# esa-prl/planning-motion_planning

Measured on AMD Instinct MI355X. Metric: Eikonal Gcells/s + ms-to-path, 4k² & 16k² costmap at 1/2/4/8 GPU, higher is better.
Workload: dtype f64; 1 GPU; C2: 4096x4096 DEM-derived cost raster, single goal, FIM on 1 MI355X; H=4096, W=4096, split=1x1, tile=64, parallelism=single-gpu

## Files before the change

planning-motion_planning_amd/csrc/eik_common.hpp:

```cpp
#pragma once
#include <hip/hip_runtime.h>
#include <stdint.h>

namespace eik {

constexpr int kTile = 64;
constexpr int kThreads = 256;
constexpr int kLds = kTile + 2;

template <typename R> struct Real;
template <> struct Real<float> {
    using U = unsigned int;
    static __host__ __device__ constexpr float inf() { return __builtin_inff(); }
};
template <> struct Real<double> {
    using U = unsigned long long;
    static __host__ __device__ constexpr double inf() { return __builtin_inf(); }
};

__device__ __forceinline__ double eik_ref(double thor, double tver, double c) {
#pragma clang fp contract(off)
    const double inf = Real<double>::inf();
    if (thor == inf) return tver == inf ? inf : tver + c;
    if (tver == inf) return thor + c;
    const double d = thor - tver;
    if (c < __builtin_fabs(d)) return __builtin_fmin(thor, tver) + c;
    return 0.5 * (thor + tver + __builtin_sqrt(2.0 * (c * c) - d * d));
}

__device__ __forceinline__ double solve3_ref(double v0, double v1, double v2, double C) {
#pragma clang fp contract(off)
    const double C2 = C * C;
    const bool m1 = v1 > v0;
    const double t01 = m1 ? v1 : v0;
    const bool m2 = v2 > t01;
    const double tmax = m2 ? v2 : t01;
    const int im = m2 ? 2 : (m1 ? 1 : 0);
    const double d0 = tmax - v0, d1 = tmax - v1, d2 = tmax - v2;
    const bool ok3 = C2 > (d0 * d0 + d1 * d1) + d2 * d2;
    const double u0 = im == 0 ? v1 : v0, u1 = im == 2 ? v1 : v2;
    const bool n1 = u1 > u0;
    const double t2 = n1 ? u1 : u0;
    const double e0 = t2 - u0, e1 = t2 - u1;
    const bool ok2 = C2 > e0 * e0 + e1 * e1;
    const double w = n1 ? u0 : u1;
    const double dw = w - w;
    const bool ok1 = C2 > dw * dw;
    double S, Q, nn;
    if (ok3) {
        S = v0 + (v1 + v2);
        Q = v0 * v0 + (v1 * v1 + v2 * v2);
        nn = 3.0;
    } else if (ok2) {
        S = u0 + u1;
        Q = u0 * u0 + u1 * u1;
        nn = 2.0;
    } else {
        S = w;
        Q = w * w;
        nn = 1.0;
    }
    const double tr = (S + __builtin_sqrt((nn * C2 + S * S) - nn * Q)) / nn;
    return (ok3 || ok2 || ok1) ? tr : Real<double>::inf();
}

template <typename R>
__device__ __forceinline__ R godunov2(R a, R b, R c) {
    const R lo = a < b ? a : b;
    const R hi = a < b ? b : a;
    const R d = hi - lo;
    const R t1 = lo + c;
    const R t2 = R(0.5) * (lo + hi + __builtin_sqrt(R(2) * (c * c) - d * d));
    return (hi == Real<R>::inf() || c < d) ? t1 : t2;
}
template <>
__device__ __forceinline__ float godunov2<float>(float a, float b, float c) {
    const float lo = fminf(a, b), hi = fmaxf(a, b);
    const float d = hi - lo;
    const float t1 = lo + c;
    const float t2 = 0.5f * (lo + hi + __builtin_amdgcn_sqrtf(2.f * (c * c) - d * d));
    return (hi == Real<float>::inf() || c < d) ? t1 : t2;
}

__device__ __forceinline__ float umin(float a, float b) {
    return __uint_as_float(min(__float_as_uint(a), __float_as_uint(b)));
}
__device__ __forceinline__ float umax(float a, float b) {
    return __uint_as_float(max(__float_as_uint(a), __float_as_uint(b)));
}
__device__ __forceinline__ double umin(double a, double b) {
    const unsigned long long x = __double_as_longlong(a), y = __double_as_longlong(b);
    return __longlong_as_double(x < y ? x : y);
}
__device__ __forceinline__ double umax(double a, double b) {
    const unsigned long long x = __double_as_longlong(a), y = __double_as_longlong(b);
    return __longlong_as_double(x < y ? y : x);
}

__device__ __forceinline__ float godunov2_step(float a, float b, float c) {
    const float lo = umin(a, b), hi = umax(a, b);
    const float d = hi - lo;
    const float t2 = lo + 0.5f * (d + __builtin_amdgcn_sqrtf(2.f * (c * c) - d * d));
    return c < d ? lo + c : t2;
}
__device__ __forceinline__ double godunov2_step(double a, double b, double c) {
    const double lo = umin(a, b), hi = umax(a, b);
    const double d = hi - lo;
    const double t2 = lo + 0.5 * (d + __builtin_sqrt(2.0 * (c * c) - d * d));
    return c < d ? lo + c : t2;
}

__device__ __forceinline__ float godunov2_fast(float a, float b, float c) {
    const float lo = umin(a, b), hi = umax(a, b);
    const float d = umin(hi - lo, c);
    const float c2 = c * c;
    const float q = __builtin_fmaf(-d, d, c2) + c2;
    return __builtin_fmaf(0.5f, d + __builtin_amdgcn_sqrtf(q), lo);
}
__device__ __forceinline__ double godunov2_fast(double a, double b, double c) {
    const double lo = umin(a, b), hi = umax(a, b);
    const double d = umin(hi - lo, c);
    const double c2 = c * c;
    const double q = __builtin_fma(-d, d, c2) + c2;
    return __builtin_fma(0.5, d + __builtin_sqrt(q), lo);
}

#ifndef EIK_CHAIN
#define EIK_CHAIN 3
#endif
__device__ __forceinline__ float godunov2_chain(float a, float b, float c, float c2x2) {
    const float lo = umin(a, b);
    const float diff = a - b;
    float d;
    asm("v_min_f32 %0, |%1|, %2" : "=v"(d) : "v"(diff), "v"(c));
    const float q = __builtin_fmaf(-d, d, c2x2);
    return __builtin_fmaf(0.5f, d + __builtin_amdgcn_sqrtf(q), lo);
}
__device__ __forceinline__ double fmin_nn(double a, double b) {
    double r;
    asm("v_min_f64 %0, %1, %2" : "=v"(r) : "v"(a), "v"(b));
    return r;
}
__device__ __forceinline__ double sqrt_sweep(double q) {
#if EIK_CHAIN
    const double qc = q;
#else
    double qc;
    asm("v_max_f64 %0, %1, %2" : "=v"(qc) : "v"(q), "v"(0x1p-1000));
#endif
    const double y = __builtin_amdgcn_rsq(qc);
    double g = qc * y, h = 0.5 * y;
    const double r = __builtin_fma(-h, g, 0.5);
    g = __builtin_fma(g, r, g);
    h = __builtin_fma(h, r, h);
    const double e = __builtin_fma(-g, g, qc);
    return __builtin_fma(e, h, g);
}
__device__ __forceinline__ double godunov2_chain(double a, double b, double c, double c2x2) {
    const double lo = fmin_nn(a, b);
    const double diff = a - b;
    double d;
    asm("v_min_f64 %0, |%1|, %2" : "=v"(d) : "v"(diff), "v"(c));
    const double q = __builtin_fma(-d, d, c2x2);
#if EIK_CHAIN >= 3
    const double base = __builtin_fma(0.5, d, lo);
    const double y = __builtin_amdgcn_rsq(q);
    const double g = q * y, h = 0.5 * y;
    const double s1 = __builtin_fma(__builtin_fma(-g, g, q), h, g);
    const double e2 = __builtin_fma(-s1, s1, q);
    return __builtin_fma(0.5, __builtin_fma(e2, h, s1), base);
#elif EIK_CHAIN >= 2
    const double base = __builtin_fma(0.5, d, lo);
    const double y = __builtin_amdgcn_rsq(q);
    const double g = q * y, h = 0.5 * y, hq = 0.25 * y;
    const double r = __builtin_fma(-h, g, 0.5);
    const double g1 = __builtin_fma(g, r, g);
    const double e = __builtin_fma(-g1, g1, q);
    return __builtin_fma(e, hq, __builtin_fma(0.5, g1, base));
#elif EIK_CHAIN
    return __builtin_fma(0.5, sqrt_sweep(q), __builtin_fma(0.5, d, lo));
#else
    return __builtin_fma(0.5, d + sqrt_sweep(q), lo);
#endif
}

__device__ __forceinline__ float wave_shr1(float v) {
    return __int_as_float(__builtin_amdgcn_update_dpp(0, __float_as_int(v), 0x138, 0xF, 0xF, false));
}
__device__ __forceinline__ float wave_shr1(float v, float lane0) {
    return __int_as_float(__builtin_amdgcn_update_dpp(__float_as_int(lane0), __float_as_int(v), 0x138, 0xF, 0xF, false));
}
__device__ __forceinline__ double wave_shr1(double v, double lane0) {
    const unsigned long long u = __double_as_longlong(v), o = __double_as_longlong(lane0);
    const int lo = __builtin_amdgcn_update_dpp((int)(o & 0xffffffffu), (int)(u & 0xffffffffu), 0x138, 0xF, 0xF, false);
    const int hi = __builtin_amdgcn_update_dpp((int)(o >> 32), (int)(u >> 32), 0x138, 0xF, 0xF, false);
    return __longlong_as_double(((unsigned long long)(unsigned)hi << 32) | (unsigned)lo);
}
__device__ __forceinline__ double wave_shr1(double v) {
    const unsigned long long u = __double_as_longlong(v);
    const int lo = __builtin_amdgcn_update_dpp(0, (int)(u & 0xffffffffu), 0x138, 0xF, 0xF, false);
    const int hi = __builtin_amdgcn_update_dpp(0, (int)(u >> 32), 0x138, 0xF, 0xF, false);
    return __longlong_as_double(((unsigned long long)(unsigned)hi << 32) | (unsigned)lo);
}

__device__ __forceinline__ float wave_shr1_umin_id(float v) {
    return __int_as_float(__builtin_amdgcn_update_dpp(-1, __float_as_int(v), 0x138, 0xF, 0xF, false));
}
__device__ __forceinline__ double wave_shr1_umin_id(double v) {
    const unsigned long long u = __double_as_longlong(v);
    const int lo = __builtin_amdgcn_update_dpp(-1, (int)(u & 0xffffffffu), 0x138, 0xF, 0xF, false);
    const int hi = __builtin_amdgcn_update_dpp(-1, (int)(u >> 32), 0x138, 0xF, 0xF, false);
    return __longlong_as_double(((unsigned long long)(unsigned)hi << 32) | (unsigned)lo);
}

__device__ __forceinline__ void lds_min(float* p, float v) {
    atomicMin(reinterpret_cast<unsigned int*>(p), __float_as_uint(v));
}
__device__ __forceinline__ void lds_min(double* p, double v) {
    atomicMin(reinterpret_cast<unsigned long long*>(p), (unsigned long long)__double_as_longlong(v));
}

}
```

planning-motion_planning_amd/csrc/fim2d.hip:

```cpp
#include "fim_engine.hpp"

namespace eik {

template <typename R>
__device__ __forceinline__ R stage_cost(R c) {
    if constexpr (sizeof(R) == 8 && EIK_CHAIN) return (c >= R(0) && c < 0x1p-500) ? R(0x1p-500) : c;
    else return c;
}

#ifndef EIK_WB_LINE
#define EIK_WB_LINE 0
#endif
#ifndef EIK_EDGE_FIRST
#define EIK_EDGE_FIRST 0
#endif

#ifndef EIK_ACT_STEP
#define EIK_ACT_STEP 0
#endif
constexpr int kActStep = EIK_ACT_STEP;



#ifndef EIK_ECOL_F64
#define EIK_ECOL_F64 1
#endif
#ifndef EIK_ECOL_F32
#define EIK_ECOL_F32 0
#endif
template <typename R>
constexpr bool kEcol = sizeof(R) == 8 ? EIK_ECOL_F64 : EIK_ECOL_F32;

#ifndef EIK_FRESH_SKIP
#define EIK_FRESH_SKIP 1
#endif
constexpr bool kFreshSkip = EIK_FRESH_SKIP;

template <typename R>
struct alignas(2 * sizeof(R)) Cell {
    R t, c;
};

#ifndef EIK_SWZ
#define EIK_SWZ 0
#endif
__device__ __forceinline__ constexpr int cell_swz(int col) { return EIK_SWZ ? (col >> 4) & 1 : 0; }
template <typename R>
__device__ __forceinline__ R& cell_t(Cell<R>* Ts, int idx, int col) {
    return reinterpret_cast<R*>(Ts + idx)[cell_swz(col)];
}
template <typename R>
__device__ __forceinline__ R& cell_c(Cell<R>* Ts, int idx, int col) {
    return reinterpret_cast<R*>(Ts + idx)[1 - cell_swz(col)];
}
template <typename R>
__device__ __forceinline__ Cell<R> make_cell(R t, R c, int col) {
    return cell_swz(col) ? Cell<R>{c, t} : Cell<R>{t, c};
}


#ifndef EIK_SWEEP_UNROLL
#define EIK_SWEEP_UNROLL 4
#endif
#ifndef EIK_SWEEP_UNROLL_F32
#define EIK_SWEEP_UNROLL_F32 8
#endif
template <typename R, int DX, int DY, bool TRACK, bool REF = false, class Hook>
__device__ __forceinline__ bool sweep_quadrant(Cell<R>* __restrict__ Ts, int lane, R keep, Hook&& hook) {
    constexpr int S = (int)sizeof(Cell<R>);
    constexpr int kRow = kLds * S;
    constexpr int D = kAhead;
    static_assert((2 * kTile) % D == 0, "pipeline depth must divide the step count");
    char* const base = reinterpret_cast<char*>(Ts);
    const int col = (DX > 0 ? lane : kTile - 1 - lane) + 1;
    constexpr int RB = (int)sizeof(R);
    const int colT = col * S + cell_swz(col) * RB;
    const int dC = (1 - 2 * cell_swz(col)) * RB;
    const int dU = (col - DX) * S + cell_swz(col - DX) * RB - colT;
    const int lo_b = -(D - 1) * kRow + colT, hi_b = (kLds - 1) * kRow + colT;
    int raw = DY > 0 ? (1 - lane) * kRow + colT : (kTile - (D - 1) + lane) * kRow + colT;
    auto off = [](int u) { return (DY > 0 ? u : D - 1 - u) * kRow; };
    auto clampb = [&](int x) {
        int r;
        asm("v_med3_i32 %0, %1, %2, %3" : "=v"(r) : "v"(x), "v"(lo_b), "v"(hi_b));
        return r;
    };
    bool changed = false;
    R cur = *reinterpret_cast<const R*>(base + (DY > 0 ? 0 : kLds - 1) * kRow + colT);
    R q_old[D], q_upx[D], q_c[D];
    int gb = clampb(raw);
    raw += DY * D * kRow;
    auto fetch = [&](int u) {
        const int o = gb + off(u);
#if EIK_SWZ
        q_old[u] = *reinterpret_cast<const R*>(base + o);
        q_c[u] = *reinterpret_cast<const R*>(base + o + dC);
#else
        const Cell<R> v = *reinterpret_cast<const Cell<R>*>(base + o);
        q_old[u] = v.t;
        q_c[u] = v.c;
#endif
        q_upx[u] = *reinterpret_cast<const R*>(base + o + dU);
    };
#pragma unroll
    for (int u = 0; u < D; ++u) fetch(u);
    constexpr int kUnroll = sizeof(R) == 8 ? EIK_SWEEP_UNROLL : EIK_SWEEP_UNROLL_F32;
#pragma unroll kUnroll
    for (int s = 0; s < 2 * kTile; s += D) {
        hook(s);
        const int gcur = gb;
        gb = clampb(raw);
        raw += DY * D * kRow;
#pragma unroll
        for (int u = 0; u < D; ++u) {
            const R c2x2 = R(2) * (q_c[u] * q_c[u]);
            R w;
            if constexpr (sizeof(R) == 8) {
                if constexpr (REF) w = eik_ref(wave_shr1(cur, q_upx[u]), cur, q_c[u]);
                else w = godunov2_chain(wave_shr1(cur, q_upx[u]), cur, q_c[u], c2x2);
                lds_min(reinterpret_cast<R*>(base + gcur + off(u)), w);
                if constexpr (TRACK) changed |= w < q_old[u] * keep;
                cur = fmin_nn(w, q_old[u]);
            } else {
                w = godunov2_chain(umin(wave_shr1_umin_id(cur), q_upx[u]), cur, q_c[u], c2x2);
                lds_min(reinterpret_cast<R*>(base + gcur + off(u)), w);
                if constexpr (TRACK) changed |= w < q_old[u] * keep;
                cur = umin(w, q_old[u]);
            }
            fetch(u);
            __builtin_amdgcn_sched_barrier(0);
        }
    }
    return changed;
}
template <typename R, int DX, int DY, bool TRACK, bool REF = false>
__device__ __forceinline__ bool sweep_quadrant(Cell<R>* __restrict__ Ts, int lane, R keep) {
    return sweep_quadrant<R, DX, DY, TRACK, REF>(Ts, lane, keep, [](int) {});
}

template <typename R>
struct TileLds {
    Cell<R> Tc[(kLds + 2 * kGuard) * kLds];
    unsigned round, flags;
    unsigned flags_acc;
    unsigned pend;
    unsigned key[5];
    int defer, tile, last;
    unsigned dirs;
    unsigned fresh;
};

template <typename R, bool COH, bool CAP = false, bool REF = false>
__device__ __forceinline__ void process_tile(const Fim2dArgs& a, int tile, TileLds<R>& L, R keep) {
    constexpr R INF = Real<R>::inf();
    Cell<R>* const Ts = L.Tc + kGuard * kLds;
    const int tid = threadIdx.x, lane = tid & 63, wave = tid >> 6;
    const int map = tile / a.tiles_per_map;
    const int rem = tile - map * a.tiles_per_map;
    const int ty = rem / a.ntx, tx = rem - (rem / a.ntx) * a.ntx;
    const R* __restrict__ cost = static_cast<const R*>(a.cost) + (int64_t)map * a.H * a.W;
    const TMem<R, COH> T(static_cast<R*>(a.T) + (int64_t)map * a.H * a.W, a.H * a.W);
    const TMem<R, COH> E(static_cast<R*>(a.ecol), (int64_t)a.capacity * 2 * kTile);
    auto eidx = [&](int t, int side, int row) { return ((int64_t)t * 2 + side) * kTile + row; };
    const int64_t y0 = (int64_t)ty * kTile, x0 = (int64_t)tx * kTile;
    const bool full = (y0 + kTile <= a.H) && (x0 + kTile <= a.W) && ((a.W & 3) == 0);
    const R capv = CAP ? (R)a.tcap[map] : INF;

    EIK_PROBE(0);
    if (tid == 0) {
        L.round = 0;
        L.flags = 0;
        L.flags_acc = 0;
        L.pend = 0;
    }
    if (tid < 5) L.key[tid] = 0x7f800000u;
    const int64_t sy = y0 + kTile < a.H ? y0 + kTile : a.H;
    const int64_t sx = x0 + kTile < a.W ? x0 + kTile : a.W;
    struct Halo {
        int h, hcol;
        int64_t hy, hx, idx;
        bool in;
    };
    auto halo_of = [&](int k) {
        Halo q;
        if (k == 0)      { q.hcol = lane + 1;            q.h = 0 * kLds + q.hcol; }
        else if (k == 1) { q.hcol = lane + 1;            q.h = (int)(sy - y0 + 1) * kLds + q.hcol; }
        else if (k == 2) { q.hcol = 0;                   q.h = (lane + 1) * kLds + q.hcol; }
        else             { q.hcol = (int)(sx - x0 + 1);  q.h = (lane + 1) * kLds + q.hcol; }
        q.hy = k == 0 ? y0 - 1 : k == 1 ? sy : y0 + lane;
        q.hx = k == 0 || k == 1 ? x0 + lane : k == 2 ? x0 - 1 : sx;
        q.in = q.hy >= 0 && q.hy < a.H && q.hx >= 0 && q.hx < a.W;
        q.idx = q.in ? q.hy * a.W + q.hx : 0;
        if (kEcol<R> && k >= 2 && q.in) q.idx = eidx(k == 2 ? tile - 1 : tile + 1, k == 2 ? 1 : 0, lane);
        return q;
    };
    auto load_halo_of = [&](const Halo& q, int k) {
        R v = kEcol<R> && k >= 2 ? E.ld(q.idx) : T.ld(q.idx);
        if (!q.in) v = load_T<R, COH>(a, T, q.hy, q.hx);
        return v;
    };
    const Halo hw = halo_of(wave);
    const int h = hw.h, hcol = hw.hcol;
    auto load_halo = [&]() { return load_halo_of(hw, wave); };
    R told[16];
    const int cx = (tid & 15) * 4;
    auto store_tile = [&](const R (&cr)[16], R hv) {
#pragma unroll
        for (int k = 0; k < 4; ++k) {
            const int ry = (tid >> 4) + 16 * k;
#pragma unroll
            for (int e = 0; e < 4; ++e)
                Ts[(ry + 1) * kLds + cx + e + 1] = make_cell<R>(told[4 * k + e], stage_cost(cr[4 * k + e]), cx + e + 1);
        }
        Ts[h] = make_cell<R>(hv, INF, hcol);
    };
    if (full && COH && kFreshSkip && __builtin_amdgcn_readfirstlane(L.fresh)) {
        R cr[16];
#pragma unroll
        for (int k = 0; k < 4; ++k) {
            const int64_t gy = y0 + (tid >> 4) + 16 * k;
            if constexpr (sizeof(R) == 4) {
                const float4 c4 = *reinterpret_cast<const float4*>(&cost[gy * a.W + x0 + cx]);
                cr[4 * k] = c4.x; cr[4 * k + 1] = c4.y; cr[4 * k + 2] = c4.z; cr[4 * k + 3] = c4.w;
            } else {
                const double2 c0 = *reinterpret_cast<const double2*>(&cost[gy * a.W + x0 + cx]);
                const double2 c1 = *reinterpret_cast<const double2*>(&cost[gy * a.W + x0 + cx + 2]);
                cr[4 * k] = c0.x; cr[4 * k + 1] = c0.y; cr[4 * k + 2] = c1.x; cr[4 * k + 3] = c1.y;
            }
#pragma unroll
            for (int e = 0; e < 4; ++e) told[4 * k + e] = INF;
        }
        store_tile(cr, load_halo());
        if (tid == 0) atomicAdd(a.visits + 2, 1ull);
    } else if (full) {
        R cr[16];
#pragma unroll
        for (int k = 0; k < 4; ++k) {
            const int64_t gy = y0 + (tid >> 4) + 16 * k;
            R tv[4];
            T.ld4(gy * a.W + x0 + cx, tv);
            if constexpr (sizeof(R) == 4) {
                const float4 c4 = *reinterpret_cast<const float4*>(&cost[gy * a.W + x0 + cx]);
                cr[4 * k] = c4.x; cr[4 * k + 1] = c4.y; cr[4 * k + 2] = c4.z; cr[4 * k + 3] = c4.w;
            } else {
                const double2 c0 = *reinterpret_cast<const double2*>(&cost[gy * a.W + x0 + cx]);
                const double2 c1 = *reinterpret_cast<const double2*>(&cost[gy * a.W + x0 + cx + 2]);
                cr[4 * k] = c0.x; cr[4 * k + 1] = c0.y; cr[4 * k + 2] = c1.x; cr[4 * k + 3] = c1.y;
            }
#pragma unroll
            for (int e = 0; e < 4; ++e) told[4 * k + e] = tv[e];
        }
        store_tile(cr, load_halo());
    } else {
        R cr[16];
#pragma unroll
        for (int k = 0; k < 4; ++k) {
            const int64_t gy = y0 + (tid >> 4) + 16 * k;
#pragma unroll
            for (int e = 0; e < 4; ++e) {
                const int64_t gx = x0 + cx + e;
                const bool in = gy < a.H && gx < a.W;
                told[4 * k + e] = load_T<R, COH>(a, T, gy, gx);
                cr[4 * k + e] = in ? cost[gy * a.W + gx] : INF;
            }
        }
        store_tile(cr, load_halo());
        if (tid < kLds) {
            if (sy - y0 < kTile) Ts[(kLds - 1) * kLds + tid] = Cell<R>{INF, INF};
            if (sx - x0 < kTile) Ts[tid * kLds + (kLds - 1)] = Cell<R>{INF, INF};
        }
    }
    if (lane < 4) cell_c(Ts, (lane >> 1) * (kLds - 1) * kLds + (lane & 1) * (kLds - 1), (lane & 1) * (kLds - 1)) = INF;
    __syncthreads();
    EIK_PROBE(1);

    unsigned dirs = L.dirs;
    int act_tile = -1;
    unsigned act_old = 0u, act_kold = 0x7f800000u;
    float act_k = 0.f;
    auto act_complete = [&]() {
        if (act_tile >= 0) qpush_complete(a, act_tile, act_old, act_k, act_kold);
        act_tile = -1;
    };
    for (int pass = 0;; ++pass) {
        auto hook = [&](int st) {
            if (EIK_ACT_SPLIT && wave == 0 && st == kActStep) act_complete();
        };
        const bool sweep = (dirs >> wave) & 1u;
        bool last_changed = false;
        if (a.max_rounds == 1) {
            if (sweep) {
                if (wave == 0)      sweep_quadrant<R, +1, +1, false, REF>(Ts, lane, keep, hook);
                else if (wave == 1) sweep_quadrant<R, -1, +1, false, REF>(Ts, lane, keep, hook);
                else if (wave == 2) sweep_quadrant<R, +1, -1, false, REF>(Ts, lane, keep, hook);
                else                sweep_quadrant<R, -1, -1, false, REF>(Ts, lane, keep, hook);
            } else {
                for (int st = 0; st < 2 * kTile; st += kAhead) hook(st);
            }
            __syncthreads();
        } else {
            for (int round = 0;; ++round) {
                bool ch = false;
                if (sweep) {
                    if (wave == 0)      ch = sweep_quadrant<R, +1, +1, true, REF>(Ts, lane, keep);
                    else if (wave == 1) ch = sweep_quadrant<R, -1, +1, true, REF>(Ts, lane, keep);
                    else if (wave == 2) ch = sweep_quadrant<R, +1, -1, true, REF>(Ts, lane, keep);
                    else                ch = sweep_quadrant<R, -1, -1, true, REF>(Ts, lane, keep);
                }
                if (__any(ch) && lane == 0) atomicOr(&L.round, 1u << (round & 31));
                __syncthreads();
                last_changed = (L.round >> (round & 31)) & 1u;
                if (!last_changed || round + 1 >= a.max_rounds) break;
            }
        }

        EIK_PROBE(2);
        unsigned pend_old = 0;
        if (COH && (a.sched & 1) && tid == 0) pend_old = atomicAnd(&a.qstate[tile], kBusy | kVisited);
        unsigned fl = 0;
        unsigned defer_rows = 0;
        R kmin_self = INF, kmin[4] = {INF, INF, INF, INF};
#pragma unroll
        for (int k = 0; k < 4; ++k) {
            const int ry = (tid >> 4) + 16 * k;
            const int64_t gy = y0 + ry;
            R nv[4];
            bool any = false;
#pragma unroll
            for (int e = 0; e < 4; ++e) {
                nv[e] = cell_t(Ts, (ry + 1) * kLds + cx + e + 1, cx + e + 1);
                any |= nv[e] < told[4 * k + e];
                if (nv[e] < told[4 * k + e] * keep && (full || (gy < a.H && x0 + cx + e < a.W))) {
                    fl |= 128u;
                    kmin_self = umin(kmin_self, nv[e]);
                    const int lx = cx + e + 1, ly = ry + 1;
                    const bool act = !CAP || nv[e] <= capv;
                    if (act && ry == 0 && nv[e] < cell_t(Ts, lx, lx)) { fl |= 1u; kmin[0] = umin(kmin[0], nv[e]); }
                    if (act && ry == kTile - 1 && nv[e] < cell_t(Ts, (kLds - 1) * kLds + lx, lx)) { fl |= 2u; kmin[1] = umin(kmin[1], nv[e]); }
                    if (act && cx + e == 0 && nv[e] < cell_t(Ts, ly * kLds, 0)) { fl |= 4u; kmin[2] = umin(kmin[2], nv[e]); }
                    if (act && cx + e == kTile - 1 && nv[e] < cell_t(Ts, ly * kLds + kLds - 1, kLds - 1)) { fl |= 8u; kmin[3] = umin(kmin[3], nv[e]); }
                    const int64_t gx = x0 + cx + e;
                    if (gy == a.H - 1 && ry != kTile - 1) fl |= 32u;
                    if (gx == a.W - 1 && cx + e != kTile - 1) fl |= 64u;
                }
            }
#if EIK_WB_LINE
            if (full) {
#pragma unroll
                for (int m = 1; m < 128 / (4 * (int)sizeof(R)); m <<= 1) any |= __shfl_xor((int)any, m) != 0;
            }
#endif
            if (any) {
                if (COH && EIK_EDGE_FIRST && full && ry != 0 && ry != kTile - 1) {
                    if (cx == 0 && nv[0] < told[4 * k]) T.st(gy * a.W + x0, nv[0]);
                    if (cx == kTile - 4 && nv[3] < told[4 * k + 3]) T.st(gy * a.W + x0 + kTile - 1, nv[3]);
                    defer_rows |= 1u << k;
                } else if (full) {
                    T.st4(gy * a.W + x0 + cx, nv);
                } else {
#pragma unroll
                    for (int e = 0; e < 4; ++e) {
                        const int64_t gx = x0 + cx + e;
                        if (gy < a.H && gx < a.W && nv[e] < told[4 * k + e]) T.st(gy * a.W + gx, nv[e]);
                    }
                }
                if (kEcol<R> && cx == 0 && nv[0] < told[4 * k]) E.st(eidx(tile, 0, ry), nv[0]);
                if (kEcol<R> && cx == kTile - 4 && nv[3] < told[4 * k + 3]) E.st(eidx(tile, 1, ry), nv[3]);
            }
            if (COH) {
#pragma unroll
                for (int e = 0; e < 4; ++e) told[4 * k + e] = nv[e];
            }
        }
        if (fl) atomicOr(&L.flags, fl);
        if (a.delta < INF || a.bctl) {
            if (kmin_self < INF) atomicMin(&L.key[0], __float_as_uint((float)kmin_self));
#pragma unroll
            for (int q = 0; q < 4; ++q)
                if (kmin[q] < INF) atomicMin(&L.key[q + 1], __float_as_uint((float)kmin[q]));
        }
        if (tid == 0) L.last = a.max_rounds == 1 ? -1 : (int)last_changed;
        if (COH && (a.sched & 1) && tid == 0) L.pend = pend_old;
        if constexpr (COH) asm volatile("s_waitcnt vmcnt(0)" ::: "memory");
        __syncthreads();
        EIK_PROBE(7);
        auto store_deferred = [&]() {
            asm volatile("" ::: "memory");
#pragma unroll
            for (int k = 0; k < 4; ++k) {
                if (defer_rows & (1u << k)) {
                    const R v[4] = {told[4 * k], told[4 * k + 1], told[4 * k + 2], told[4 * k + 3]};
                    T.st4((y0 + (tid >> 4) + 16 * k) * a.W + x0 + cx, v);
                }
            }
        };
        if (COH) {
            const unsigned f = L.flags;
            const unsigned pend = L.pend & (kPending | kFromN | kFromS | kFromW | kFromE);
            const bool self = (f & 128u) != 0u;
            if ((!self && !pend) || pass + 1 >= a.max_passes || a.max_rounds != 1) {
                store_deferred();
                break;
            }
            const R hv = load_halo();
            if (tid == 64) charge_inplace_pass(a);
            const bool defer = (a.sched & 2) && pass > 0;
            if constexpr (EIK_ACT_SPLIT)
                act_tile = activate_neighbours_issue(a, tile, defer ? 0u : f, act_old, L.key, act_k,
                                                     act_kold);
            else
                activate_neighbours(a, tile, defer ? 0u : f, L.key, 0, 0u);
            if (defer && tid == 0) L.flags_acc |= f & 0x6fu;
            dirs = self ? 0xFu : sweep_dirs(pend);
            cell_t(Ts, h, hcol) = hv;
            store_deferred();
            __syncthreads();
            if (tid == 0) {
                L.flags = 0;
                L.pend = 0;
            }
        } else {
            break;
        }
    }
    act_complete();
    EIK_PROBE(3);
}

template <typename R>
__device__ __forceinline__ void activate_after(const Fim2dArgs& a, int tile, const TileLds<R>& L, int list,
                                               unsigned stamp) {
    const unsigned f = L.flags;
    activate_neighbours(a, tile, f | L.flags_acc, L.key, list, stamp);
    if (threadIdx.x == 0) {
        const bool self = L.last < 0 ? (f & 128u) != 0u : L.last != 0;
        if (a.mode == kModePersistent) {
            const unsigned p = L.pend & (kFromN | kFromS | kFromW | kFromE);
            if (self || (L.pend & kPending)) {
                if (self && a.bctl) atomicMin(&a.key[tile], 0u);
                atomicOr(&a.qstate[tile], kPending | (self ? kSelf : p));
            }
        } else if (self) {
            enqueue(a, tile, list, stamp, __uint_as_float(L.key[0]));
        }
    }
}

template <typename R>
__device__ __forceinline__ void init_guard_rows(TileLds<R>& L) {
    const int tid = threadIdx.x;
    for (int i = tid; i < kGuard * kLds; i += kThreads) {
        L.Tc[i] = Cell<R>{Real<R>::inf(), Real<R>::inf()};
        L.Tc[(kLds + kGuard) * kLds + i] = Cell<R>{Real<R>::inf(), Real<R>::inf()};
    }
}

template <typename R>
__global__ __launch_bounds__(kThreads) void fim2d_sweep_kernel(Fim2dArgs a) {
    constexpr R INF = Real<R>::inf();
    __shared__ TileLds<R> L;
    const int tid = threadIdx.x;
    init_guard_rows(L);
    const int cur = a.iter % 3, nxt = (a.iter + 1) % 3, rst = (a.iter + 2) % 3;
    const int cnt = a.counts[cur];
    if (blockIdx.x == 0 && tid == 0) {
        a.counts[rst] = 0;
        a.minkey[rst] = 0x7f800000u;
    }
    const unsigned stamp = a.iter + 2;
    const float thr = __uint_as_float(a.minkey[cur]) + a.delta;
    const R keep = (R)a.keep;
    if (tid == 0) L.dirs = 0xFu;

    for (int it = blockIdx.x; it < cnt; it += gridDim.x) {
        const int tile = a.lists[(int64_t)cur * a.capacity + it];
        if (a.delta < INF) {
            if (tid == 0) {
                const float k = __uint_as_float(atomicOr(&a.key[tile], 0u));
                L.defer = k > thr;
                if (k > thr) enqueue(a, tile, nxt, stamp, k);
                else atomicExch(&a.key[tile], 0x7f800000u);
            }
            __syncthreads();
            const bool defer = L.defer;
            __syncthreads();
            if (defer) continue;
        }
        process_tile<R, false>(a, tile, L, keep);
        activate_after(a, tile, L, nxt, stamp);
        if (tid == 0 && a.visits) atomicAdd(a.visits, 1ull);
        __syncthreads();
    }
}

template <typename R>
__device__ __forceinline__ void merge_strip_cells(const Fim2dArgs& a, int side, const R* rv, R* g, int64_t i,
                                                  int64_t len, unsigned* count) {
    R v = Real<R>::inf();
    bool drop = false;
    if (i < len) {
        v = ld_system(rv + i);
        drop = v < ld_agent(g + i);
        if (drop) st_scoped(g + i, v, __HIP_MEMORY_SCOPE_AGENT);
    }
    const unsigned long long m = __ballot(drop);
    if (!m) return;
    __builtin_amdgcn_fence(__ATOMIC_RELEASE, "agent");
    unsigned k = drop ? __float_as_uint((float)v) : 0x7f800000u;
#pragma unroll
    for (int d = 32; d > 0; d >>= 1) k = min(k, (unsigned)__shfl_xor((int)k, d));
    if ((threadIdx.x & 63) == (unsigned)__builtin_ctzll(m)) {
        if (count) atomicAdd(count, (unsigned)__popcll(m));
        int ty, tx;
        if (side < 2) {
            tx = (int)(i / kTile);
            ty = side == 0 ? 0 : a.nty - 1;
        } else {
            ty = (int)(i / kTile);
            tx = side == 2 ? 0 : a.ntx - 1;
        }
        activate(a, ty * a.ntx + tx, a.iter % 3, a.iter + 1, __uint_as_float(k), kFromN << side);
    }
}

template <typename R>
__device__ __forceinline__ void live_agent(const Fim2dArgs& a, unsigned* sh) {
    const int tid = threadIdx.x;
    auto pack = [&](unsigned par, bool skip_busy) {
        const R* T = static_cast<const R*>(a.T);
        R* tg[4];
        for (int k = 0; k < 4; ++k) tg[k] = static_cast<R*>(a.live->send[par][k]);
        auto idle = [&](int64_t ty, int64_t tx) {
            return !skip_busy ||
                   (__hip_atomic_load(&a.qstate[ty * a.ntx + tx], __ATOMIC_RELAXED, __HIP_MEMORY_SCOPE_AGENT) &
                    (kPending | kBusy)) == 0u;
        };
        for (int64_t i = tid; i < a.W; i += blockDim.x) {
            if (tg[0] && idle(0, i / kTile)) st_scoped(tg[0] + i, ld_agent(T + i), __HIP_MEMORY_SCOPE_SYSTEM);
            if (tg[1] && idle(a.nty - 1, i / kTile))
                st_scoped(tg[1] + i, ld_agent(T + (a.H - 1) * a.W + i), __HIP_MEMORY_SCOPE_SYSTEM);
        }
        for (int64_t i = tid; i < a.H; i += blockDim.x) {
            if (tg[2] && idle(i / kTile, 0)) st_scoped(tg[2] + i, ld_agent(T + i * a.W), __HIP_MEMORY_SCOPE_SYSTEM);
            if (tg[3] && idle(i / kTile, a.ntx - 1))
                st_scoped(tg[3] + i, ld_agent(T + i * a.W + a.W - 1), __HIP_MEMORY_SCOPE_SYSTEM);
        }
    };
    auto merge = [&](unsigned par, unsigned* count) {
        for (int side = 0; side < 4; ++side) {
            const R* rv = static_cast<const R*>(a.live->recv[par][side]);
            R* g = static_cast<R*>(const_cast<void*>(a.ghost[side]));
            if (!rv || !g) continue;
            const int64_t len = side < 2 ? a.W : a.H;
            for (int64_t i0 = 0; i0 < len; i0 += blockDim.x) merge_strip_cells<R>(a, side, rv, g, i0 + tid, len, count);
        }
    };
    live_agent_loop(a, sh, pack, merge);
}

template <typename R, int WPS, bool CAP = false, bool REF = false>
__global__ __launch_bounds__(kThreads, WPS) void fim2d_persist_kernel(Fim2dArgs a) {
    __shared__ TileLds<R> L;
    if (a.live && blockIdx.x == 0) {
        __shared__ unsigned sh[4];
        live_agent<R>(a, sh);
        return;
    }
    init_guard_rows(L);
    EIK_KSTART();
    const R keep = (R)a.keep;
    int tile = -1;
    unsigned nvis = 0;
    for (;;) {
        if (EIK_EDGE_FIRST && tile >= 0) {
            asm volatile("s_waitcnt vmcnt(0)" ::: "memory");
            __syncthreads();
        }
        if (threadIdx.x < 64) {
            if (tile >= 0) {
                EIK_PROBE(4);
                activate_after(a, tile, L, 0, 0u);
                asm volatile("s_waitcnt vmcnt(0)" ::: "memory");
                if (threadIdx.x == 0) {
                    qfinish(a, tile);
                    if (++nvis == 64u) {
                        charge_visits(a, 64ull);
                        nvis = 0;
                    }
                }
            }
            EIK_PROBE(5);
        } else if (threadIdx.x < 128 && (a.bctl || threadIdx.x == 64)) {
            unsigned trig = 0;
            const int t = a.bctl ? qgrab_prio(a, trig) : qgrab(a, trig);
            if (threadIdx.x == 64) {
                L.tile = t;
                L.dirs = sweep_dirs(trig);
                L.fresh = !(trig & kVisited);
                if (t >= 0) EIK_VISIT(t, trig, L.dirs);
            }
        }
        __syncthreads();
        EIK_PROBE(6);
        tile = __builtin_amdgcn_readfirstlane(L.tile);
        if (tile < 0) break;
        process_tile<R, true, CAP, REF>(a, tile, L, keep);
    }
    if (threadIdx.x == 0 && nvis) atomicAdd(a.visits, (unsigned long long)nvis);
}
template <typename R>
__global__ void fim2d_init_kernel(R* __restrict__ T, int64_t n, unsigned* __restrict__ mark, int64_t ntiles,
                                  unsigned* __restrict__ key, unsigned* __restrict__ minkey, unsigned* __restrict__ qstate,
                                  unsigned* __restrict__ qslot, int64_t nslots, unsigned* __restrict__ counts,
                                  unsigned* __restrict__ qctl, unsigned* __restrict__ visits, unsigned* __restrict__ edge,
                                  R* __restrict__ ecol) {
    const int64_t stride = (int64_t)gridDim.x * blockDim.x;
    if (blockIdx.x == 0 && threadIdx.x < kQueueCtlBytes / 4) {
        const int t = threadIdx.x;
        if (qctl) qctl[t] = 0u;
        if (t < 4) {
            if (counts) counts[t] = 0u;
            if (edge) edge[t] = 0u;
        }
        if (t < 22 && visits) visits[t] = 0u;
    }
    for (int64_t i = (int64_t)blockIdx.x * blockDim.x + threadIdx.x; i < n; i += stride) T[i] = Real<R>::inf();
    if (ecol)
        for (int64_t i = (int64_t)blockIdx.x * blockDim.x + threadIdx.x; i < ntiles * 2 * kTile; i += stride)
            ecol[i] = Real<R>::inf();
    for (int64_t i = (int64_t)blockIdx.x * blockDim.x + threadIdx.x; i < ntiles; i += stride) {
        mark[i] = 0;
        key[i] = 0x7f800000u;
        if (qstate) qstate[i] = 0;
    }
    for (int64_t i = (int64_t)blockIdx.x * blockDim.x + threadIdx.x; i < nslots; i += stride) qslot[i] = 0;
    if (blockIdx.x == 0 && threadIdx.x < 3) minkey[threadIdx.x] = threadIdx.x == 0 ? 0u : 0x7f800000u;
}

template <typename R>
__global__ void fim2d_seed_kernel(Fim2dArgs a, const int64_t* __restrict__ goals, int nmaps) {
    const int m = blockIdx.x * blockDim.x + threadIdx.x;
    if (m == 0) {
        a.counts[1] = 0;
        a.counts[2] = 0;
    }
    if (m >= nmaps) return;
    const int64_t gx = goals[2 * m], gy = goals[2 * m + 1];
    if (gx < 0 || gy < 0 || gx >= a.W || gy >= a.H) return;
    static_cast<R*>(a.T)[(int64_t)m * a.H * a.W + gy * a.W + gx] = R(0);
    const int tile = m * a.tiles_per_map + (int)(gy / kTile) * a.ntx + (int)(gx / kTile);
    if (kEcol<R> && a.ecol && (gx % kTile == 0 || gx % kTile == kTile - 1))
        static_cast<R*>(a.ecol)[((int64_t)tile * 2 + (gx % kTile == 0 ? 0 : 1)) * kTile + gy % kTile] = R(0);
    if (a.mode == kModePersistent) {
        qpush(a, tile, kSelf | kVisited);
        return;
    }
    a.mark[tile] = 1;
    a.key[tile] = 0u;
    const int pos = atomicAdd(&a.counts[0], 1);
    a.lists[pos] = tile;
}

template <typename R>
__global__ __launch_bounds__(256) void prio_delta_kernel(const R* __restrict__ cost, int64_t n, float mult,
                                                          float* __restrict__ out) {
    __shared__ double ssum[4];
    __shared__ int scnt[4];
    double sum = 0.0;
    int cnt = 0;
    for (int i = threadIdx.x; i < 4096; i += 256) {
        const unsigned long long hsh = (unsigned long long)(i + 1) * 0x9E3779B97F4A7C15ull;
        const double c = (double)cost[(int64_t)((hsh >> 11) % (unsigned long long)n)];
        if (c > 0.0 && c < Real<double>::inf()) {
            sum += log(c);
            ++cnt;
        }
    }
    for (int d = 32; d > 0; d >>= 1) {
        sum += __shfl_down(sum, d);
        cnt += __shfl_down(cnt, d);
    }
    if ((threadIdx.x & 63) == 0) {
        ssum[threadIdx.x >> 6] = sum;
        scnt[threadIdx.x >> 6] = cnt;
    }
    __syncthreads();
    if (threadIdx.x == 0) {
        const double s = ssum[0] + ssum[1] + ssum[2] + ssum[3];
        const int c = scnt[0] + scnt[1] + scnt[2] + scnt[3];
        const double g = c ? exp(s / c) : 1.0;
        *out = (float)(mult * 64.0 * g > 1e-30 ? mult * 64.0 * g : 1e-30);
    }
}

hipError_t fim2d_prio_delta(const void* cost, bool f64, int64_t n, float mult, float* out, hipStream_t st) {
    if (f64)
        hipLaunchKernelGGL(prio_delta_kernel<double>, dim3(1), dim3(256), 0, st, static_cast<const double*>(cost), n,
                           mult, out);
    else
        hipLaunchKernelGGL(prio_delta_kernel<float>, dim3(1), dim3(256), 0, st, static_cast<const float*>(cost), n,
                           mult, out);
    return hipGetLastError();
}

__global__ void fim2d_qrewind_kernel(Fim2dArgs a) {
    if (a.bctl) {
        const int64_t stride = (int64_t)gridDim.x * blockDim.x;
        for (int64_t i = (int64_t)blockIdx.x * blockDim.x + threadIdx.x; i <= (int64_t)a.qmask; i += stride) {
            const unsigned v = a.qslot[i];
            if (v == 0u) continue;
            const unsigned tag = v >> kBandTagShift;
            if (tag) atomicAnd(&a.bmem[(v & kSlotTileMask) - 1u], ~(1ull << (tag - 1u)));
            a.qslot[i] = 0u;
        }
    }
    if (blockIdx.x == 0 && threadIdx.x == 0) *a.qhead = *a.qtail;
}
static void launch_qrewind(const Fim2dArgs& a, hipStream_t st) {
    const int grid = a.bctl ? (int)std::min<int64_t>(256, ((int64_t)a.qmask + 256) / 256) : 1;
    hipLaunchKernelGGL(fim2d_qrewind_kernel, dim3(grid), dim3(a.bctl ? 256 : 1), 0, st, a);
}

template <typename R>
__global__ __launch_bounds__(256) void fim2d_merge_ghost_kernel(Fim2dArgs a, int side, const R* __restrict__ recv,
                                                                int64_t len) {
    R* g = static_cast<R*>(const_cast<void*>(a.ghost[side]));
    merge_strip_cells<R>(a, side, recv, g, (int64_t)blockIdx.x * blockDim.x + threadIdx.x, len, nullptr);
}

template <typename R>
__global__ void fim2d_pack_edges_kernel(Fim2dArgs a, R* __restrict__ n, R* __restrict__ s, R* __restrict__ w,
                                        R* __restrict__ e) {
    const int64_t i = (int64_t)blockIdx.x * blockDim.x + threadIdx.x;
    const R* T = static_cast<const R*>(a.T);
    if (i < a.W) {
        if (n) st_scoped(n + i, ld_agent(T + i), __HIP_MEMORY_SCOPE_SYSTEM);
        if (s) st_scoped(s + i, ld_agent(T + (a.H - 1) * a.W + i), __HIP_MEMORY_SCOPE_SYSTEM);
    }
    if (i < a.H) {
        if (w) st_scoped(w + i, ld_agent(T + i * a.W), __HIP_MEMORY_SCOPE_SYSTEM);
        if (e) st_scoped(e + i, ld_agent(T + i * a.W + a.W - 1), __HIP_MEMORY_SCOPE_SYSTEM);
    }
}

hipError_t fim2d_sweep(const Fim2dArgs& a, bool f64, int grid, hipStream_t st) {
    if (f64)
        hipLaunchKernelGGL(fim2d_sweep_kernel<double>, dim3(grid), dim3(kThreads), 0, st, a);
    else
        hipLaunchKernelGGL(fim2d_sweep_kernel<float>, dim3(grid), dim3(kThreads), 0, st, a);
    return hipGetLastError();
}

int fim2d_persist_resident(bool f64, int cus, bool wide) {
    int per_cu = 0;
    const hipError_t e =
        f64    ? hipOccupancyMaxActiveBlocksPerMultiprocessor(&per_cu, fim2d_persist_kernel<double, 1>, kThreads, 0)
        : wide ? hipOccupancyMaxActiveBlocksPerMultiprocessor(&per_cu, fim2d_persist_kernel<float, 4>, kThreads, 0)
               : hipOccupancyMaxActiveBlocksPerMultiprocessor(&per_cu, fim2d_persist_kernel<float, 1>, kThreads, 0);
    if (e != hipSuccess || per_cu < 1) per_cu = 1;
    return per_cu * cus;
}

hipError_t fim2d_persist(const Fim2dArgs& a, bool f64, int grid, hipStream_t st, bool wide, bool rewind) {
    if (f64 && a.ref_arith && a.tcap)
        hipLaunchKernelGGL((fim2d_persist_kernel<double, 1, true, true>), dim3(grid), dim3(kThreads), 0, st, a);
    else if (f64 && a.ref_arith)
        hipLaunchKernelGGL((fim2d_persist_kernel<double, 1, false, true>), dim3(grid), dim3(kThreads), 0, st, a);
    else if (f64 && a.tcap)
        hipLaunchKernelGGL((fim2d_persist_kernel<double, 1, true>), dim3(grid), dim3(kThreads), 0, st, a);
    else if (f64)
        hipLaunchKernelGGL((fim2d_persist_kernel<double, 1>), dim3(grid), dim3(kThreads), 0, st, a);
    else if (wide)
        hipLaunchKernelGGL((fim2d_persist_kernel<float, 4>), dim3(grid), dim3(kThreads), 0, st, a);
    else
        hipLaunchKernelGGL((fim2d_persist_kernel<float, 1>), dim3(grid), dim3(kThreads), 0, st, a);
    if (rewind) launch_qrewind(a, st);
    return hipGetLastError();
}

hipError_t fim2d_qrewind(const Fim2dArgs& a, hipStream_t st) {
    launch_qrewind(a, st);
    return hipGetLastError();
}

hipError_t fim2d_init(const Fim2dArgs& a, bool f64, int nmaps, const int64_t* d_goals, unsigned* edge, hipStream_t st) {
    static_assert(kQueueCtlBytes / 4 <= 256, "the init kernel's block 0 clears the queue words");
    const int64_t n = (int64_t)nmaps * a.H * a.W;
    const int64_t ntiles = (int64_t)nmaps * a.tiles_per_map;
    const int grid = (int)std::min<int64_t>(4096, (n + 255) / 256);
    const int64_t nslots = a.qslot ? (int64_t)a.qmask + 1 : 0;
    unsigned* const counts = reinterpret_cast<unsigned*>(a.counts);
    unsigned* const qctl = reinterpret_cast<unsigned*>(a.qhead);
    unsigned* const visits = reinterpret_cast<unsigned*>(a.visits);
    if (f64) {
        hipLaunchKernelGGL(fim2d_init_kernel<double>, dim3(grid), dim3(256), 0, st, static_cast<double*>(a.T), n,
                           a.mark, ntiles, a.key, a.minkey, a.qstate, a.qslot, nslots, counts, qctl, visits, edge,
                           kEcol<double> ? static_cast<double*>(a.ecol) : nullptr);
        hipLaunchKernelGGL(fim2d_seed_kernel<double>, dim3((nmaps + 255) / 256), dim3(256), 0, st, a, d_goals, nmaps);
    } else {
        hipLaunchKernelGGL(fim2d_init_kernel<float>, dim3(grid), dim3(256), 0, st, static_cast<float*>(a.T), n,
                           a.mark, ntiles, a.key, a.minkey, a.qstate, a.qslot, nslots, counts, qctl, visits, edge,
                           kEcol<float> ? static_cast<float*>(a.ecol) : nullptr);
        hipLaunchKernelGGL(fim2d_seed_kernel<float>, dim3((nmaps + 255) / 256), dim3(256), 0, st, a, d_goals, nmaps);
    }
    return hipGetLastError();
}

hipError_t fim2d_merge_ghost(const Fim2dArgs& a, bool f64, int side, const void* recv, int64_t len, hipStream_t st) {
    const int grid = (int)((len + 255) / 256);
    if (f64)
        hipLaunchKernelGGL(fim2d_merge_ghost_kernel<double>, dim3(grid), dim3(256), 0, st, a, side,
                           static_cast<const double*>(recv), len);
    else
        hipLaunchKernelGGL(fim2d_merge_ghost_kernel<float>, dim3(grid), dim3(256), 0, st, a, side,
                           static_cast<const float*>(recv), len);
    return hipGetLastError();
}

hipError_t fim2d_pack_edges(const Fim2dArgs& a, bool f64, void* n, void* s, void* w, void* e, hipStream_t st) {
    const int64_t len = a.H > a.W ? a.H : a.W;
    const int grid = (int)((len + 255) / 256);
    if (f64)
        hipLaunchKernelGGL(fim2d_pack_edges_kernel<double>, dim3(grid), dim3(256), 0, st, a, (double*)n, (double*)s,
                           (double*)w, (double*)e);
    else
        hipLaunchKernelGGL(fim2d_pack_edges_kernel<float>, dim3(grid), dim3(256), 0, st, a, (float*)n, (float*)s,
                           (float*)w, (float*)e);
    return hipGetLastError();
}

}
```

Measured before the change: 7.820 Gcells/s.

## Restructure tile writeback: wave-level DPP reductions for flags/keys, edge checks by boundary lanes

Rewrites the tile-change detection after each FIM sweep. All 16 cell values are loaded into registers first and changed cells are recorded in a bitmask. Only boundary lanes check halo neighbours, and flags and key minima are combined with a DPP wave reduction before a single LDS atomic per wave, instead of per-thread atomics. The qstate atomicAnd is moved after the stores, and launch-bound waves per SIMD are raised for the default WPS. The disabled WB_LINE and EDGE_FIRST deferred-store paths are removed. The higher occupancy target and the 16-value register array may increase register pressure or cause spills.

```diff
diff --git a/planning-motion_planning_amd/csrc/eik_common.hpp b/planning-motion_planning_amd/csrc/eik_common.hpp
--- a/planning-motion_planning_amd/csrc/eik_common.hpp
+++ b/planning-motion_planning_amd/csrc/eik_common.hpp
@@ -213,6 +213,19 @@
     return __longlong_as_double(((unsigned long long)(unsigned)hi << 32) | (unsigned)lo);
 }
 
+template <class Op>
+__device__ __forceinline__ unsigned wave_reduce_idem(unsigned v, Op op) {
+#define EIK_DPP_STEP(ctrl, rows) v = op(v, (unsigned)__builtin_amdgcn_update_dpp((int)v, (int)v, ctrl, rows, 0xF, false))
+    EIK_DPP_STEP(0xB1, 0xF);
+    EIK_DPP_STEP(0x4E, 0xF);
+    EIK_DPP_STEP(0x141, 0xF);
+    EIK_DPP_STEP(0x140, 0xF);
+    EIK_DPP_STEP(0x142, 0xA);
+    EIK_DPP_STEP(0x143, 0xC);
+#undef EIK_DPP_STEP
+    return (unsigned)__builtin_amdgcn_readlane((int)v, 63);
+}
+
 __device__ __forceinline__ void lds_min(float* p, float v) {
     atomicMin(reinterpret_cast<unsigned int*>(p), __float_as_uint(v));
 }
diff --git a/planning-motion_planning_amd/csrc/fim2d.hip b/planning-motion_planning_amd/csrc/fim2d.hip
--- a/planning-motion_planning_amd/csrc/fim2d.hip
+++ b/planning-motion_planning_amd/csrc/fim2d.hip
@@ -8,12 +8,6 @@
     else return c;
 }
 
-#ifndef EIK_WB_LINE
-#define EIK_WB_LINE 0
-#endif
-#ifndef EIK_EDGE_FIRST
-#define EIK_EDGE_FIRST 0
-#endif
 
 #ifndef EIK_ACT_STEP
 #define EIK_ACT_STEP 0
@@ -273,6 +267,7 @@
     if (lane < 4) cell_c(Ts, (lane >> 1) * (kLds - 1) * kLds + (lane & 1) * (kLds - 1), (lane & 1) * (kLds - 1)) = INF;
     __syncthreads();
     EIK_PROBE(1);
+    if constexpr (CAP) asm volatile("" ::"v"(capv));
 
     unsigned dirs = L.dirs;
     int act_tile = -1;
@@ -316,92 +311,106 @@
 
         EIK_PROBE(2);
         unsigned pend_old = 0;
-        if (COH && (a.sched & 1) && tid == 0) pend_old = atomicAnd(&a.qstate[tile], kBusy | kVisited);
-        unsigned fl = 0;
-        unsigned defer_rows = 0;
-        R kmin_self = INF, kmin[4] = {INF, INF, INF, INF};
+        R nv[16];
+#pragma unroll
+        for (int k = 0; k < 4; ++k) {
+            const int ry = (tid >> 4) + 16 * k;
+#pragma unroll
+            for (int e = 0; e < 4; ++e) nv[4 * k + e] = cell_t(Ts, (ry + 1) * kLds + cx + e + 1, cx + e + 1);
+        }
+        unsigned chg = 0;
 #pragma unroll
         for (int k = 0; k < 4; ++k) {
             const int ry = (tid >> 4) + 16 * k;
             const int64_t gy = y0 + ry;
-            R nv[4];
             bool any = false;
 #pragma unroll
             for (int e = 0; e < 4; ++e) {
-                nv[e] = cell_t(Ts, (ry + 1) * kLds + cx + e + 1, cx + e + 1);
-                any |= nv[e] < told[4 * k + e];
-                if (nv[e] < told[4 * k + e] * keep && (full || (gy < a.H && x0 + cx + e < a.W))) {
-                    fl |= 128u;
-                    kmin_self = umin(kmin_self, nv[e]);
-                    const int lx = cx + e + 1, ly = ry + 1;
-                    const bool act = !CAP || nv[e] <= capv;
-                    if (act && ry == 0 && nv[e] < cell_t(Ts, lx, lx)) { fl |= 1u; kmin[0] = umin(kmin[0], nv[e]); }
-                    if (act && ry == kTile - 1 && nv[e] < cell_t(Ts, (kLds - 1) * kLds + lx, lx)) { fl |= 2u; kmin[1] = umin(kmin[1], nv[e]); }
-                    if (act && cx + e == 0 && nv[e] < cell_t(Ts, ly * kLds, 0)) { fl |= 4u; kmin[2] = umin(kmin[2], nv[e]); }
-                    if (act && cx + e == kTile - 1 && nv[e] < cell_t(Ts, ly * kLds + kLds - 1, kLds - 1)) { fl |= 8u; kmin[3] = umin(kmin[3], nv[e]); }
-                    const int64_t gx = x0 + cx + e;
-                    if (gy == a.H - 1 && ry != kTile - 1) fl |= 32u;
-                    if (gx == a.W - 1 && cx + e != kTile - 1) fl |= 64u;
-                }
-            }
-#if EIK_WB_LINE
-            if (full) {
-#pragma unroll
-                for (int m = 1; m < 128 / (4 * (int)sizeof(R)); m <<= 1) any |= __shfl_xor((int)any, m) != 0;
-            }
-#endif
+                const int i = 4 * k + e;
+                any |= nv[i] < told[i];
+                const bool in = full || (gy < a.H && x0 + cx + e < a.W);
+                chg |= (nv[i] < told[i] * keep && in) ? 1u << i : 0u;
+            }
             if (any) {
-                if (COH && EIK_EDGE_FIRST && full && ry != 0 && ry != kTile - 1) {
-                    if (cx == 0 && nv[0] < told[4 * k]) T.st(gy * a.W + x0, nv[0]);
-                    if (cx == kTile - 4 && nv[3] < told[4 * k + 3]) T.st(gy * a.W + x0 + kTile - 1, nv[3]);
-                    defer_rows |= 1u << k;
-                } else if (full) {
-                    T.st4(gy * a.W + x0 + cx, nv);
+                if (full) {
+                    const R v[4] = {nv[4 * k], nv[4 * k + 1], nv[4 * k + 2], nv[4 * k + 3]};
+                    T.st4(gy * a.W + x0 + cx, v);
                 } else {
 #pragma unroll
                     for (int e = 0; e < 4; ++e) {
                         const int64_t gx = x0 + cx + e;
-                        if (gy < a.H && gx < a.W && nv[e] < told[4 * k + e]) T.st(gy * a.W + gx, nv[e]);
+                        if (gy < a.H && gx < a.W && nv[4 * k + e] < told[4 * k + e]) T.st(gy * a.W + gx, nv[4 * k + e]);
                     }
                 }
-                if (kEcol<R> && cx == 0 && nv[0] < told[4 * k]) E.st(eidx(tile, 0, ry), nv[0]);
-                if (kEcol<R> && cx == kTile - 4 && nv[3] < told[4 * k + 3]) E.st(eidx(tile, 1, ry), nv[3]);
-            }
-            if (COH) {
-#pragma unroll
-                for (int e = 0; e < 4; ++e) told[4 * k + e] = nv[e];
-            }
-        }
-        if (fl) atomicOr(&L.flags, fl);
-        if (a.delta < INF || a.bctl) {
-            if (kmin_self < INF) atomicMin(&L.key[0], __float_as_uint((float)kmin_self));
-#pragma unroll
-            for (int q = 0; q < 4; ++q)
-                if (kmin[q] < INF) atomicMin(&L.key[q + 1], __float_as_uint((float)kmin[q]));
+                if (kEcol<R> && cx == 0 && nv[4 * k] < told[4 * k]) E.st(eidx(tile, 0, ry), nv[4 * k]);
+                if (kEcol<R> && cx == kTile - 4 && nv[4 * k + 3] < told[4 * k + 3]) E.st(eidx(tile, 1, ry), nv[4 * k + 3]);
+            }
+        }
+        if (COH && (a.sched & 1) && tid == 0)
+            pend_old = atomicAnd(&a.qstate[tile + (int)__builtin_amdgcn_mbcnt_lo(0u, 0u)], kBusy | kVisited);
+        __builtin_amdgcn_sched_barrier(0);
+        if (COH) {
+#pragma unroll
+            for (int i = 0; i < 16; ++i) told[i] = nv[i];
+        }
+        const bool keys = a.delta < INF || a.bctl;
+        unsigned fl = chg ? 128u : 0u;
+        R kmin_self = INF, kmin[4] = {INF, INF, INF, INF};
+        if (keys) {
+#pragma unroll
+            for (int i = 0; i < 16; ++i) kmin_self = umin(kmin_self, (chg >> i) & 1u ? nv[i] : INF);
+        }
+        auto edge = [&](int q, int i0, int di, int h0, int dh, int hc) {
+            R hv[4];
+#pragma unroll
+            for (int j = 0; j < 4; ++j) hv[j] = cell_t(Ts, h0 + dh * j, hc < 0 ? cx + j + 1 : hc);
+#pragma unroll
+            for (int j = 0; j < 4; ++j) {
+                const int i = i0 + di * j;
+                const bool act = !CAP || nv[i] <= capv;
+                const bool hit = ((chg >> i) & 1u) && act && nv[i] < hv[j];
+                fl |= hit ? 1u << q : 0u;
+                kmin[q] = umin(kmin[q], hit ? nv[i] : INF);
+            }
+        };
+        const int ly0 = (tid >> 4) + 1;
+        if ((tid >> 4) == 0) edge(0, 0, 1, cx + 1, 1, -1);
+        if ((tid >> 4) == 15) edge(1, 12, 1, (kLds - 1) * kLds + cx + 1, 1, -1);
+        if ((tid & 15) == 0) edge(2, 0, 4, ly0 * kLds, 16 * kLds, 0);
+        if ((tid & 15) == 15) edge(3, 3, 4, ly0 * kLds + kLds - 1, 16 * kLds, kLds - 1);
+        if (!full) {
+#pragma unroll
+            for (int k = 0; k < 4; ++k) {
+                const int ry = (tid >> 4) + 16 * k;
+                if (y0 + ry == a.H - 1 && ry != kTile - 1 && ((chg >> (4 * k)) & 0xFu)) fl |= 32u;
+            }
+#pragma unroll
+            for (int e = 0; e < 4; ++e)
+                if (x0 + cx + e == a.W - 1 && cx + e != kTile - 1 && (chg & (0x1111u << e))) fl |= 64u;
+        }
+        const unsigned wfl = wave_reduce_idem(fl, [](unsigned x, unsigned y) { return x | y; });
+        if (wfl && lane == 0) atomicOr(&L.flags, wfl);
+        if (keys) {
+            const R km[5] = {kmin_self, kmin[0], kmin[1], kmin[2], kmin[3]};
+#pragma unroll
+            for (int q = 0; q < 5; ++q) {
+                const unsigned wk = wave_reduce_idem(__float_as_uint((float)km[q]), [](unsigned x, unsigned y) { return min(x, y); });
+                if (wk < 0x7f800000u && lane == 0) atomicMin(&L.key[q], wk);
+            }
         }
         if (tid == 0) L.last = a.max_rounds == 1 ? -1 : (int)last_changed;
+        if constexpr (COH) {
+            __builtin_amdgcn_s_waitcnt(0x0F70);
+            asm volatile("s_waitcnt vmcnt(0)" ::: "memory");
+        }
         if (COH && (a.sched & 1) && tid == 0) L.pend = pend_old;
-        if constexpr (COH) asm volatile("s_waitcnt vmcnt(0)" ::: "memory");
         __syncthreads();
         EIK_PROBE(7);
-        auto store_deferred = [&]() {
-            asm volatile("" ::: "memory");
-#pragma unroll
-            for (int k = 0; k < 4; ++k) {
-                if (defer_rows & (1u << k)) {
-                    const R v[4] = {told[4 * k], told[4 * k + 1], told[4 * k + 2], told[4 * k + 3]};
-                    T.st4((y0 + (tid >> 4) + 16 * k) * a.W + x0 + cx, v);
-                }
-            }
-        };
         if (COH) {
             const unsigned f = L.flags;
             const unsigned pend = L.pend & (kPending | kFromN | kFromS | kFromW | kFromE);
             const bool self = (f & 128u) != 0u;
-            if ((!self && !pend) || pass + 1 >= a.max_passes || a.max_rounds != 1) {
-                store_deferred();
-                break;
-            }
+            if ((!self && !pend) || pass + 1 >= a.max_passes || a.max_rounds != 1) break;
             const R hv = load_halo();
             if (tid == 64) charge_inplace_pass(a);
             const bool defer = (a.sched & 2) && pass > 0;
@@ -413,7 +422,6 @@
             if (defer && tid == 0) L.flags_acc |= f & 0x6fu;
             dirs = self ? 0xFu : sweep_dirs(pend);
             cell_t(Ts, h, hcol) = hv;
-            store_deferred();
             __syncthreads();
             if (tid == 0) {
                 L.flags = 0;
@@ -558,8 +566,10 @@
     live_agent_loop(a, sh, pack, merge);
 }
 
+template <typename R, int WPS, bool REF>
+constexpr int kPersistWaves = WPS > 1 ? WPS : sizeof(R) == 4 ? 3 : REF ? 1 : 2;
 template <typename R, int WPS, bool CAP = false, bool REF = false>
-__global__ __launch_bounds__(kThreads, WPS) void fim2d_persist_kernel(Fim2dArgs a) {
+__global__ __launch_bounds__(kThreads, (kPersistWaves<R, WPS, REF>)) void fim2d_persist_kernel(Fim2dArgs a) {
     __shared__ TileLds<R> L;
     if (a.live && blockIdx.x == 0) {
         __shared__ unsigned sh[4];
@@ -572,10 +582,6 @@
     int tile = -1;
     unsigned nvis = 0;
     for (;;) {
-        if (EIK_EDGE_FIRST && tile >= 0) {
-            asm volatile("s_waitcnt vmcnt(0)" ::: "memory");
-            __syncthreads();
-        }
         if (threadIdx.x < 64) {
             if (tile >= 0) {
                 EIK_PROBE(4);
```

After: 8.591 Gcells/s, median of 6. 1.1x the previous value.
